# VinAIResearch/Point-Unet

Hardware: AMD Instinct MI355X
Metric: points_per_sec_forward (higher is better)
Workload: dtype f32

## Files before the change

### point-unet_amd/csrc/attpool32b.hip

```cpp
#include "attpool.h"
#include "b3_ops.h"
#include "mfma_tile.h"
#include "wave_ops.h"

namespace ps {

struct Att32bArgs {
    const float* xyz;
    const int32_t* idx;
    const int32_t* order;
    const float* fg;
    const uint4* w1; const float* b1;
    const uint4* w2; const float* b2;
    const uint4* wb;
    float* agg;
    int n_total, n_cloud;
};

__device__ __forceinline__ B3Planes load_planes(const uint4* img, int slot, int lane)
{
    B3Planes r;
    r.p[0] = img[(slot * 3 + 0) * 64 + lane];
    r.p[1] = img[(slot * 3 + 1) * 64 + lane];
    r.p[2] = img[(slot * 3 + 2) * 64 + lane];
    return r;
}

template <int D, int STAGE, int KN, int WAVES>
__global__ __launch_bounds__(WAVES * 64) void att32b_kernel(Att32bArgs a)
{
    constexpr int H = D / 2, LDF = H + D, PITCH = H + 4, PPT = 32 / KN, RP = 16 / PPT;
    constexpr int CBH = H / 32, CBD = D / 32, NQ = H / 16;
    constexpr int W1Q = CBH * 3 * 64, W2Q = STAGE == 2 ? CBH * NQ * 3 * 64 : 0, WBQ = CBD * NQ * 3 * 64;
    constexpr int TILE = 32 * PITCH;
    static_assert(H % 32 == 0 && (KN == 16 || KN == 32), "att32b: d_out >= 64, K in {16, 32}");

    extern __shared__ __attribute__((aligned(16))) float smem[];
    const int wave = __builtin_amdgcn_readfirstlane(threadIdx.x >> 6), lane = threadIdx.x & 63;
    const int hl = lane >> 5, c32 = lane & 31;
    uint4* Wq = reinterpret_cast<uint4*>(smem);
    constexpr int WTOT = (W1Q + W2Q + WBQ) * 4 + 2 * H;
    float* own = smem + WTOT + wave * (32 + TILE);
    int* NB = reinterpret_cast<int*>(own);
    float* T1 = own + 32;
    for (int i = threadIdx.x; i < W1Q; i += WAVES * 64) Wq[i] = a.w1[i];
    for (int i = threadIdx.x; i < W2Q; i += WAVES * 64) Wq[W1Q + i] = a.w2[i];
    for (int i = threadIdx.x; i < WBQ; i += WAVES * 64) Wq[W1Q + W2Q + i] = a.wb[i];
    float* bias = smem + (W1Q + W2Q + WBQ) * 4;
    for (int i = threadIdx.x; i < H; i += WAVES * 64) {
        bias[i] = a.b1[i];
        bias[H + i] = STAGE == 2 ? a.b2[i] : 0.f;
    }
    __syncthreads();
    const uint4 *w1 = Wq, *w2 = Wq + W1Q, *wb = Wq + W1Q + W2Q;
    const float *b1 = bias, *b2 = bias + H;

    const int per_xcd = ((((a.n_total + 7) >> 3) + PPT - 1) / PPT) * PPT;
    const int xcd = blockIdx.x & 7, slot = blockIdx.x >> 3, slots = gridDim.x >> 3;
    const int t_end = min(a.n_total, (xcd + 1) * per_xcd);
    const int t_first = xcd * per_xcd + (slot * WAVES + wave) * PPT, t_step = slots * WAVES * PPT;
    int n_pp[PPT], n_nl = 0;
    float n_c[3], n_n[3];
    const bool one_cloud = a.n_total == a.n_cloud;
    auto cloud_base = [&](int row) { return one_cloud ? 0 : (row / a.n_cloud) * a.n_cloud; };
    auto gstage = [&](int st, int t0n) {
        if (t0n >= t_end) return;
        if (st == 0) {
#pragma unroll
            for (int i = 0; i < PPT; ++i) {
                const int t = min(t0n + i, t_end - 1);
                n_pp[i] = a.order ? cloud_base(t) + a.order[t] : t;
            }
        } else if (st == 1) {
            const unsigned p = PPT == 2 ? (c32 >= KN ? n_pp[PPT - 1] : n_pp[0]) : n_pp[0];
            n_nl = a.idx[p * (unsigned)KN + (unsigned)(c32 & (KN - 1))];
            const float* cp = a.xyz + 3u * p;
            n_c[0] = cp[0]; n_c[1] = cp[1]; n_c[2] = cp[2];
        } else {
            const int p = PPT == 2 ? (c32 >= KN ? n_pp[PPT - 1] : n_pp[0]) : n_pp[0];
            n_nl += cloud_base(p);
            const float* np = a.xyz + 3u * (unsigned)n_nl;
            n_n[0] = np[0]; n_n[1] = np[1]; n_n[2] = np[2];
        }
    };
    gstage(0, t_first);
    gstage(1, t_first);
    gstage(2, t_first);
    for (int t0 = t_first; t0 < t_end; t0 += t_step) {
        int pp[PPT];
#pragma unroll
        for (int i = 0; i < PPT; ++i) pp[i] = n_pp[i];
        const int nbr = n_nl;
        const float cx = n_c[0], cy = n_c[1], cz = n_c[2];
        const float nx = n_n[0], ny = n_n[1], nz = n_n[2];
        const float rx = cx - nx, ry = cy - ny, rz = cz - nz;
        const float dis = __builtin_amdgcn_sqrtf(rx * rx + ry * ry + rz * rz);
        const float ev[8] = {hl ? ny : dis, hl ? nz : rx, hl ? 0.f : ry, hl ? 0.f : rz, hl ? 0.f : cx, hl ? 0.f : cy, hl ? 0.f : cz, hl ? 0.f : nx};
        const B3Planes E = b3_split8<3>(ev);
        if (hl == 0) NB[c32] = nbr;
        gstage(0, t0 + t_step);
        wave_lds_sync();
        unsigned off[16];
        {
            const unsigned col0 = (unsigned)c32 * 4u;
#pragma unroll
            for (int g4 = 0; g4 < 4; ++g4) {
                const int4 nb4 = *reinterpret_cast<const int4*>(NB + 8 * g4 + 4 * hl);
                off[4 * g4] = __umul24(nb4.x, LDF * 4u) + col0; off[4 * g4 + 1] = __umul24(nb4.y, LDF * 4u) + col0;
                off[4 * g4 + 2] = __umul24(nb4.z, LDF * 4u) + col0; off[4 * g4 + 3] = __umul24(nb4.w, LDF * 4u) + col0;
            }
        }
        const char* fgb = reinterpret_cast<const char*>(a.fg);
        f32x2 gq[2][8], v[2][8];
        auto gather = [&](int i, f32x2 (&gdst)[8], f32x2 (&vdst)[8]) {
            const int rel = i * 32 * 4;
#pragma unroll
            for (int r = 0; r < 16; ++r) gdst[r >> 1][r & 1] = *reinterpret_cast<const float*>(fgb + off[r] + (rel + H * 4));
            if (i * 32 < H) {
#pragma unroll
                for (int r = 0; r < 16; ++r) vdst[r >> 1][r & 1] = *reinterpret_cast<const float*>(fgb + off[r] + rel);
            }
        };
        gather(0, gq[0], v[0]);

        f32x16 f1[CBH];
#pragma unroll
        for (int cb = 0; cb < CBH; ++cb) {
            f32x16 acc;
#pragma unroll
            for (int g4 = 0; g4 < 4; ++g4) {
                const float4 bb = *reinterpret_cast<const float4*>(b1 + cb * 32 + g4 * 8 + hl * 4);
                acc[4 * g4] = bb.x; acc[4 * g4 + 1] = bb.y; acc[4 * g4 + 2] = bb.z; acc[4 * g4 + 3] = bb.w;
            }
            acc = b3_mfma6<3>(load_planes(w1, cb, lane), E, acc);
#pragma unroll
            for (int r = 0; r < 16; ++r) f1[cb][r] = leaky02(acc[r]);
        }
        gstage(1, t0 + t_step);
        B3Planes P[NQ];
        auto split_block = [&](const f32x16& f, B3Planes& lo, B3Planes& hi) {
            const float x0[8] = {f[0], f[1], f[2], f[3], f[4], f[5], f[6], f[7]};
            const float x1[8] = {f[8], f[9], f[10], f[11], f[12], f[13], f[14], f[15]};
            lo = b3_split8<3>(x0);
            hi = b3_split8<3>(x1);
        };
        auto store_block = [&](const f32x16& f, int cb) {
#pragma unroll
            for (int g4 = 0; g4 < 4; ++g4) {
                float4 o;
                o.x = f[4 * g4]; o.y = f[4 * g4 + 1]; o.z = f[4 * g4 + 2]; o.w = f[4 * g4 + 3];
                *reinterpret_cast<float4*>(T1 + c32 * PITCH + cb * 32 + g4 * 8 + hl * 4) = o;
            }
        };
#pragma unroll
        for (int cb = 0; cb < CBH; ++cb) split_block(f1[cb], P[2 * cb], P[2 * cb + 1]);
        if constexpr (STAGE == 1) {
#pragma unroll
            for (int cb = 0; cb < CBH; ++cb) store_block(f1[cb], cb);
        } else {
            f32x16 f2[CBH];
#pragma unroll
            for (int cb = 0; cb < CBH; ++cb) {
                f32x16 acc;
#pragma unroll
                for (int g4 = 0; g4 < 4; ++g4) {
                    const float4 bb = *reinterpret_cast<const float4*>(b2 + cb * 32 + g4 * 8 + hl * 4);
                    acc[4 * g4] = bb.x; acc[4 * g4 + 1] = bb.y; acc[4 * g4 + 2] = bb.z; acc[4 * g4 + 3] = bb.w;
                }
#pragma unroll
                for (int q = 0; q < NQ; ++q) acc = b3_mfma6<3>(load_planes(w2, cb * NQ + q, lane), P[q], acc);
#pragma unroll
                for (int r = 0; r < 16; ++r) f2[cb][r] = leaky02(acc[r]);
            }
#pragma unroll
            for (int cb = 0; cb < CBH; ++cb) {
                split_block(f2[cb], P[2 * cb], P[2 * cb + 1]);
                store_block(f2[cb], cb);
            }
        }
        wave_lds_sync();
        const float* TX = T1;

#pragma unroll
        for (int cb = 0; cb < CBD; ++cb) {
            if (cb + 1 < CBD) gather(cb + 1, gq[(cb + 1) & 1], v[(cb + 1) & 1]);
            if (cb == 0) gstage(2, t0 + t_step);
            f32x16 acc;
#pragma unroll
            for (int r = 0; r < 16; ++r) acc[r] = 0.f;
#pragma unroll
            for (int q = 0; q < NQ; ++q) acc = b3_mfma6<3>(P[q], load_planes(wb, cb * NQ + q, lane), acc);
            f32x2 (&vv)[8] = v[cb & 1];
            if (cb * 32 >= H) {
                const float* tv = TX + (cb * 32 - H + c32) + 4 * hl * PITCH;
#pragma unroll
                for (int r = 0; r < 16; ++r) vv[r >> 1][r & 1] = tv[((r & 3) + 8 * (r >> 2)) * PITCH];
            }
            f32x2 sc[8];
            const f32x2 l2e = {1.4426950408889634f, 1.4426950408889634f};
#pragma unroll
            for (int j = 0; j < 8; ++j) sc[j] = __builtin_elementwise_fma(gq[cb & 1][j], l2e, f32x2{acc[2 * j], acc[2 * j + 1]});
            constexpr int PP = RP / 2;
#pragma unroll
            for (int pi = 0; pi < PPT; ++pi) {
                float m = fmaxf(sc[pi * PP][0], sc[pi * PP][1]);
#pragma unroll
                for (int j = 1; j < PP; ++j) m = fmaxf(m, fmaxf(sc[pi * PP + j][0], sc[pi * PP + j][1]));
                m = swap32_max(m);
                const f32x2 mm = {m, m};
                f32x2 ssum2 = {0.f, 0.f}, num2 = {0.f, 0.f};
#pragma unroll
                for (int j = 0; j < PP; ++j) {
                    const f32x2 dd = sc[pi * PP + j] - mm;
                    const f32x2 ex = {__builtin_amdgcn_exp2f(dd[0]), __builtin_amdgcn_exp2f(dd[1])};
                    ssum2 += ex;
                    num2 = __builtin_elementwise_fma(ex, vv[pi * PP + j], num2);
                }
                const float ssum = swap32_sum(ssum2[0] + ssum2[1]);
                const float num = swap32_sum(num2[0] + num2[1]);
                if (hl == 0 && t0 + pi < t_end) a.agg[__umul24(pp[pi], D) + (unsigned)(cb * 32 + c32)] = num * __builtin_amdgcn_rcpf(ssum);
            }
        }
        wave_lds_sync();
    }
}


template <int D, int STAGE, int KN, int WAVES>
__global__ __launch_bounds__(WAVES * 64) void att32s_kernel(Att32bArgs a)
{
    constexpr int H = D / 2, LDF = H + D, PITCH = H + 4, PPT = 32 / KN, RP = 16 / PPT;
    constexpr int CBH = H / 32, CBD = D / 32, NQ = H / 16;
    constexpr int PLQ = NQ * 3 * 64;
    constexpr int NB_H = CBH / WAVES, NB_D = CBD / WAVES;
    static_assert(CBH % WAVES == 0 && NB_D == 2 && (KN == 16 || KN == 32), "att32s: two score blocks per wave");

    extern __shared__ __attribute__((aligned(16))) float smem[];
    const int wave = threadIdx.x >> 6, lane = threadIdx.x & 63;
    const int hl = lane >> 5, c32 = lane & 31;
    int* NB = reinterpret_cast<int*>(smem);
    uint4* PA = reinterpret_cast<uint4*>(smem + 32);
    uint4* PB = STAGE == 2 ? PA + PLQ : PA;
    float* TV = reinterpret_cast<float*>(PB + PLQ);

    const int per_xcd = ((((a.n_total + 7) >> 3) + PPT - 1) / PPT) * PPT;
    const int xcd = blockIdx.x & 7, slot = blockIdx.x >> 3, slots = gridDim.x >> 3;
    const int t_end = min(a.n_total, (xcd + 1) * per_xcd);
    const int t_first = xcd * per_xcd + slot * PPT, t_step = slots * PPT;
    int n_pp[PPT], n_nl = 0;
    float n_c[3], n_n[3];
    const bool one_cloud = a.n_total == a.n_cloud;
    auto cloud_base = [&](int row) { return one_cloud ? 0 : (row / a.n_cloud) * a.n_cloud; };
    auto gstage = [&](int st, int t0n) {
        if (t0n >= t_end) return;
        if (st == 0) {
#pragma unroll
            for (int i = 0; i < PPT; ++i) {
                const int t = min(t0n + i, t_end - 1);
                n_pp[i] = a.order ? cloud_base(t) + a.order[t] : t;
            }
        } else if (st == 1) {
            const unsigned p = PPT == 2 ? (c32 >= KN ? n_pp[PPT - 1] : n_pp[0]) : n_pp[0];
            n_nl = a.idx[p * (unsigned)KN + (unsigned)(c32 & (KN - 1))];
            const float* cp = a.xyz + 3u * p;
            n_c[0] = cp[0]; n_c[1] = cp[1]; n_c[2] = cp[2];
        } else {
            const int p = PPT == 2 ? (c32 >= KN ? n_pp[PPT - 1] : n_pp[0]) : n_pp[0];
            n_nl += cloud_base(p);
            const float* np = a.xyz + 3u * (unsigned)n_nl;
            n_n[0] = np[0]; n_n[1] = np[1]; n_n[2] = np[2];
        }
    };
    auto seed = [&](const float* b, int cb) {
        f32x16 acc;
#pragma unroll
        for (int g4 = 0; g4 < 4; ++g4) {
            const float4 bb = *reinterpret_cast<const float4*>(b + cb * 32 + g4 * 8 + hl * 4);
            acc[4 * g4] = bb.x; acc[4 * g4 + 1] = bb.y; acc[4 * g4 + 2] = bb.z; acc[4 * g4 + 3] = bb.w;
        }
        return acc;
    };
    auto emit_block = [&](const f32x16& acc, int cb, uint4* planes, bool values) {
        float x0[8], x1[8];
#pragma unroll
        for (int r = 0; r < 8; ++r) { x0[r] = leaky02(acc[r]); x1[r] = leaky02(acc[8 + r]); }
        const B3Planes lo = b3_split8<3>(x0), hi = b3_split8<3>(x1);
#pragma unroll
        for (int pl = 0; pl < 3; ++pl) {
            planes[((2 * cb) * 3 + pl) * 64 + lane] = lo.p[pl];
            planes[((2 * cb + 1) * 3 + pl) * 64 + lane] = hi.p[pl];
        }
        if (values) {
#pragma unroll
            for (int g4 = 0; g4 < 4; ++g4) {
                const float* x = g4 < 2 ? x0 + 4 * g4 : x1 + 4 * (g4 - 2);
                *reinterpret_cast<float4*>(TV + c32 * PITCH + cb * 32 + g4 * 8 + hl * 4) = make_float4(x[0], x[1], x[2], x[3]);
            }
        }
    };
    gstage(0, t_first);
    gstage(1, t_first);
    gstage(2, t_first);
    static_assert(NB_H == 1, "att32s: one transposed block per wave");
    const B3Planes W1 = load_planes(a.w1, wave, lane);
    const f32x16 seed1 = seed(a.b1, wave);
    constexpr int PD = D >= 512 ? 4 : 2;
    constexpr int PD2 = STAGE == 2 ? (D >= 512 ? 4 : 8) : 1;
    const int cbA = wave, cbB = wave + WAVES;
    for (int t0 = t_first; t0 < t_end; t0 += t_step) {
        int pp[PPT];
#pragma unroll
        for (int i = 0; i < PPT; ++i) pp[i] = n_pp[i];
        const int nbr = n_nl;
        const float cx = n_c[0], cy = n_c[1], cz = n_c[2];
        const float nx = n_n[0], ny = n_n[1], nz = n_n[2];
        const float rx = cx - nx, ry = cy - ny, rz = cz - nz;
        const float dis = __builtin_amdgcn_sqrtf(rx * rx + ry * ry + rz * rz);
        const float ev[8] = {hl ? ny : dis, hl ? nz : rx, hl ? 0.f : ry, hl ? 0.f : rz, hl ? 0.f : cx, hl ? 0.f : cy, hl ? 0.f : cz, hl ? 0.f : nx};
        const B3Planes E = b3_split8<3>(ev);
        if (hl == 0 && wave == 0) NB[c32] = nbr;
        gstage(0, t0 + t_step);
        B3Planes ring[PD2], rA[PD], rB[PD];
        if constexpr (STAGE == 2) {
#pragma unroll
            for (int q = 0; q < PD2; ++q) ring[q] = load_planes(a.w2, wave * NQ + q, lane);
        } else {
#pragma unroll
            for (int q = 0; q < PD; ++q) {
                rA[q] = load_planes(a.wb, cbA * NQ + q, lane);
                rB[q] = load_planes(a.wb, cbB * NQ + q, lane);
            }
        }

        emit_block(b3_mfma6<3>(W1, E, seed1), wave, PA, STAGE == 1);
        __syncthreads();
        gstage(1, t0 + t_step);
        unsigned off[16];
        {
            const unsigned col0 = (unsigned)(wave * 32 + c32) * 4u;
#pragma unroll
            for (int g4 = 0; g4 < 4; ++g4) {
                const int4 nb4 = *reinterpret_cast<const int4*>(NB + 8 * g4 + 4 * hl);
                off[4 * g4] = __umul24(nb4.x, LDF * 4u) + col0; off[4 * g4 + 1] = __umul24(nb4.y, LDF * 4u) + col0;
                off[4 * g4 + 2] = __umul24(nb4.z, LDF * 4u) + col0; off[4 * g4 + 3] = __umul24(nb4.w, LDF * 4u) + col0;
            }
        }
        const char* fgb = reinterpret_cast<const char*>(a.fg);
        if constexpr (STAGE == 2) {
            const int cb = wave;
            f32x16 acc = seed(a.b2, cb);
#pragma unroll 1
            for (int q0 = 0; q0 + PD2 < NQ; q0 += PD2) {
#pragma unroll
                for (int j = 0; j < PD2; ++j) {
                    acc = b3_mfma6<3>(ring[j], load_planes(PA, q0 + j, lane), acc);
                    ring[j] = load_planes(a.w2, cb * NQ + q0 + j + PD2, lane);
                }
            }
#pragma unroll
            for (int j = 0; j < PD2; ++j) acc = b3_mfma6<3>(ring[j], load_planes(PA, NQ - PD2 + j, lane), acc);
#pragma unroll
            for (int q = 0; q < PD; ++q) {
                rA[q] = load_planes(a.wb, cbA * NQ + q, lane);
                rB[q] = load_planes(a.wb, cbB * NQ + q, lane);
            }
            emit_block(acc, cb, PB, true);
            __syncthreads();
        }
        gstage(2, t0 + t_step);

        f32x16 accA, accB;
#pragma unroll
        for (int r = 0; r < 16; ++r) { accA[r] = 0.f; accB[r] = 0.f; }
        f32x2 gq[2][8], v[2][8];
        {
#pragma unroll 1
            for (int q0 = 0; q0 + PD < NQ; q0 += PD) {
#pragma unroll
                for (int j = 0; j < PD; ++j) {
                    const B3Planes x = load_planes(PB, q0 + j, lane);
                    accA = b3_mfma6<3>(x, rA[j], accA);
                    accB = b3_mfma6<3>(x, rB[j], accB);
                    rA[j] = load_planes(a.wb, cbA * NQ + q0 + j + PD, lane);
                    rB[j] = load_planes(a.wb, cbB * NQ + q0 + j + PD, lane);
                }
            }
#pragma unroll
            for (int i = 0; i < 2; ++i)
#pragma unroll
                for (int r = 0; r < 16; ++r) gq[i][r >> 1][r & 1] = *reinterpret_cast<const float*>(fgb + off[r] + (i * WAVES * 32 * 4 + H * 4));
#pragma unroll
            for (int j = 0; j < PD; ++j) {
                const B3Planes x = load_planes(PB, NQ - PD + j, lane);
                accA = b3_mfma6<3>(x, rA[j], accA);
                accB = b3_mfma6<3>(x, rB[j], accB);
            }
        }
#pragma unroll
        for (int r = 0; r < 16; ++r) v[0][r >> 1][r & 1] = *reinterpret_cast<const float*>(fgb + off[r]);
#pragma unroll
        for (int ii = 0; ii < 2; ++ii) {
            const int i = 1 - ii;
            const int cb = wave + i * WAVES;
            const f32x16& acc = i == 0 ? accA : accB;
            f32x2 (&vv)[8] = v[i];
            if (cb * 32 >= H) {
                const float* tv = TV + (cb * 32 - H + c32) + 4 * hl * PITCH;
#pragma unroll
                for (int r = 0; r < 16; ++r) vv[r >> 1][r & 1] = tv[((r & 3) + 8 * (r >> 2)) * PITCH];
            }
            f32x2 sc[8];
            const f32x2 l2e = {1.4426950408889634f, 1.4426950408889634f};
#pragma unroll
            for (int j = 0; j < 8; ++j) sc[j] = __builtin_elementwise_fma(gq[i][j], l2e, f32x2{acc[2 * j], acc[2 * j + 1]});
            constexpr int PP = RP / 2;
#pragma unroll
            for (int pi = 0; pi < PPT; ++pi) {
                float m = fmaxf(sc[pi * PP][0], sc[pi * PP][1]);
#pragma unroll
                for (int j = 1; j < PP; ++j) m = fmaxf(m, fmaxf(sc[pi * PP + j][0], sc[pi * PP + j][1]));
                m = swap32_max(m);
                const f32x2 mm = {m, m};
                f32x2 ssum2 = {0.f, 0.f}, num2 = {0.f, 0.f};
#pragma unroll
                for (int j = 0; j < PP; ++j) {
                    const f32x2 dd = sc[pi * PP + j] - mm;
                    const f32x2 ex = {__builtin_amdgcn_exp2f(dd[0]), __builtin_amdgcn_exp2f(dd[1])};
                    ssum2 += ex;
                    num2 = __builtin_elementwise_fma(ex, vv[pi * PP + j], num2);
                }
                const float ssum = swap32_sum(ssum2[0] + ssum2[1]);
                const float num = swap32_sum(num2[0] + num2[1]);
                if (hl == 0 && t0 + pi < t_end) a.agg[__umul24(pp[pi], D) + (unsigned)(cb * 32 + c32)] = num * __builtin_amdgcn_rcpf(ssum);
            }
        }
        __syncthreads();
    }
}

static inline int kmap(int q, int g, int j)
{
    const int r = 8 * (q & 1) + j;
    return 32 * (q >> 1) + (r & 3) + 8 * (r >> 2) + 4 * g;
}

void pack_b3(const float* W, int cin, int cout, uint16_t* out)
{
    const int nq = cin / 16, cbs = cout / 32;
    for (int cb = 0; cb < cbs; ++cb)
        for (int q = 0; q < nq; ++q)
            for (int pl = 0; pl < 3; ++pl)
                for (int l = 0; l < 64; ++l)
                    for (int j = 0; j < 8; ++j)
                        out[(((((size_t)cb * nq + q) * 3 + pl) * 64 + l) * 8) + j] = b3_piece_of(W[(size_t)kmap(q, l >> 5, j) * cout + 32 * cb + (l & 31)], pl);
}

void pack_b3_locse(const float* W1, int cout, uint16_t* out)
{
    const int cbs = cout / 32;
    for (int cb = 0; cb < cbs; ++cb)
        for (int pl = 0; pl < 3; ++pl)
            for (int l = 0; l < 64; ++l)
                for (int j = 0; j < 8; ++j) {
                    const int k = 8 * (l >> 5) + j;
                    out[((((size_t)cb * 3 + pl) * 64 + l) * 8) + j] = k < 10 ? b3_piece_of(W1[(size_t)k * cout + 32 * cb + (l & 31)], pl) : (uint16_t)0;
                }
}

template <int D, int STAGE, int KN>
static int launch_att32b(ps_context* c, const Att32bArgs& a)
{
    constexpr int H = D / 2, PITCH = H + 4, TILE = 32 * PITCH;
    constexpr int CBH = H / 32, CBD = D / 32, NQ = H / 16;
    constexpr int WAVES = D == 128 ? 8 : (STAGE == 1 ? 16 : 12);
    constexpr int PER_CU = 1;
    constexpr size_t planes = (size_t)(CBH + (STAGE == 2 ? CBH * NQ : 0) + CBD * NQ) * 3 * 64 * 16;
    constexpr size_t smem = planes + sizeof(float) * (2 * H + (size_t)WAVES * (32 + TILE));
    static_assert(smem <= 160 * 1024, "att32b: weights + tiles exceed the LDS");
    auto kern = att32b_kernel<D, STAGE, KN, WAVES>;
    PS_HIP(hipFuncSetAttribute(reinterpret_cast<const void*>(kern), hipFuncAttributeMaxDynamicSharedMemorySize, (int)smem));
    const int tiles = ceil_div(a.n_total, 32 / KN);
    const int blocks = (std::min(ceil_div(tiles, WAVES), 256 * PER_CU) + 7) & ~7;
    hipLaunchKernelGGL(kern, dim3(blocks), dim3(WAVES * 64), smem, c->stream, a);
    PS_HIP(hipGetLastError());
    return PS_OK;
}

template <int D, int STAGE, int KN>
static int launch_att32s(ps_context* c, const Att32bArgs& a)
{
    constexpr int H = D / 2, PITCH = H + 4, NQ = H / 16;
    constexpr int WAVES = D / 64;
    constexpr size_t smem = sizeof(float) * 32 + (size_t)(STAGE == 2 ? 2 : 1) * NQ * 3 * 64 * 16 + sizeof(float) * 32 * PITCH;
    static_assert(smem <= 160 * 1024, "att32s: planes + value tile exceed the LDS");
    auto kern = att32s_kernel<D, STAGE, KN, WAVES>;
    if (smem > 48 * 1024) PS_HIP(hipFuncSetAttribute(reinterpret_cast<const void*>(kern), hipFuncAttributeMaxDynamicSharedMemorySize, (int)smem));
    const int tiles = ceil_div(a.n_total, 32 / KN);
    const int blocks = (std::min(tiles, 256 * 16) + 7) & ~7;
    hipLaunchKernelGGL(kern, dim3(blocks), dim3(WAVES * 64), smem, c->stream, a);
    PS_HIP(hipGetLastError());
    return PS_OK;
}

bool att_pool32b_fits(const AttStage& s)
{
    return att_pool32_fits(s) && s.p32->w1b && (s.d == 64 || s.d == 128 || s.d == 256 || s.d == 512);
}

int att_pool32b_stage(ps_context* c, const AttStage& s)
{
    Att32bArgs a;
    a.xyz = s.xyz; a.idx = s.idx; a.order = s.order; a.fg = s.fg;
    a.w1 = reinterpret_cast<const uint4*>(s.p32->w1b); a.b1 = s.lfa1->bias;
    a.w2 = s.lfa2 ? reinterpret_cast<const uint4*>(s.p32->w2b) : nullptr; a.b2 = s.lfa2 ? s.lfa2->bias : nullptr;
    a.wb = reinterpret_cast<const uint4*>(s.lfa2 ? s.p32->wb2b : s.p32->wb1b);
    a.agg = s.agg;
    a.n_total = (int)s.n_total; a.n_cloud = (int)s.n_cloud;
    if (s.n_total <= 0) return PS_OK;
    const int stage = s.lfa2 ? 2 : 1;
#define PS_A32B(DD)                                                                                                      \
    if (s.k == 16) return stage == 1 ? launch_att32b<DD, 1, 16>(c, a) : launch_att32b<DD, 2, 16>(c, a);                  \
    return stage == 1 ? launch_att32b<DD, 1, 32>(c, a) : launch_att32b<DD, 2, 32>(c, a)
    if (s.d == 64) { PS_A32B(64); }
    if (s.d == 128) { PS_A32B(128); }
#undef PS_A32B
#define PS_A32S(DD)                                                                                                      \
    if (s.k == 16) return stage == 1 ? launch_att32s<DD, 1, 16>(c, a) : launch_att32s<DD, 2, 16>(c, a);                  \
    return stage == 1 ? launch_att32s<DD, 1, 32>(c, a) : launch_att32s<DD, 2, 32>(c, a)
    if (s.d == 256) { PS_A32S(256); }
    PS_A32S(512);
#undef PS_A32S
}

}
```

Measured before the change: 193.5 million.

## Process two point tiles per iteration in att32s to reuse weight planes

The att32s attention-pool kernel now handles T (default 2) point tiles per loop iteration, so each weight plane loaded from global memory feeds MFMAs for several tiles. The per-block value tile is replaced by a small per-wave scratch that transposes values into registers, and the separate second plane buffer is dropped. Neighbour gathers are interleaved with the softmax/aggregation work. Launch bounds now request two blocks per CU and the grid is sized per XCD group. The cost is higher register pressure from doubled accumulators and more LDS for per-tile planes.

```diff
diff --git a/point-unet_amd/csrc/attpool32b.hip b/point-unet_amd/csrc/attpool32b.hip
--- a/point-unet_amd/csrc/attpool32b.hip
+++ b/point-unet_amd/csrc/attpool32b.hip
@@ -226,10 +226,10 @@
 }
 
 
-template <int D, int STAGE, int KN, int WAVES>
-__global__ __launch_bounds__(WAVES * 64) void att32s_kernel(Att32bArgs a)
-{
-    constexpr int H = D / 2, LDF = H + D, PITCH = H + 4, PPT = 32 / KN, RP = 16 / PPT;
+template <int D, int STAGE, int KN, int WAVES, int T>
+__global__ __launch_bounds__(WAVES * 64, 2) void att32s_kernel(Att32bArgs a)
+{
+    constexpr int H = D / 2, LDF = H + D, SCP = 36, PPT = 32 / KN, RP = 16 / PPT;
     constexpr int CBH = H / 32, CBD = D / 32, NQ = H / 16;
     constexpr int PLQ = NQ * 3 * 64;
     constexpr int NB_H = CBH / WAVES, NB_D = CBD / WAVES;
@@ -239,36 +239,47 @@
     const int wave = threadIdx.x >> 6, lane = threadIdx.x & 63;
     const int hl = lane >> 5, c32 = lane & 31;
     int* NB = reinterpret_cast<int*>(smem);
-    uint4* PA = reinterpret_cast<uint4*>(smem + 32);
-    uint4* PB = STAGE == 2 ? PA + PLQ : PA;
-    float* TV = reinterpret_cast<float*>(PB + PLQ);
+    uint4* PA = reinterpret_cast<uint4*>(smem + T * 32);
+    float* SC = reinterpret_cast<float*>(PA + T * PLQ) + wave * (32 * SCP);
 
     const int per_xcd = ((((a.n_total + 7) >> 3) + PPT - 1) / PPT) * PPT;
     const int xcd = blockIdx.x & 7, slot = blockIdx.x >> 3, slots = gridDim.x >> 3;
     const int t_end = min(a.n_total, (xcd + 1) * per_xcd);
-    const int t_first = xcd * per_xcd + slot * PPT, t_step = slots * PPT;
-    int n_pp[PPT], n_nl = 0;
-    float n_c[3], n_n[3];
+    const int t_first = xcd * per_xcd + slot * (T * PPT), t_step = slots * (T * PPT);
+    int n_pp[T][PPT], n_nl[T];
+    float n_c[T][3], n_n[T][3];
+#pragma unroll
+    for (int u = 0; u < T; ++u) {
+        n_nl[u] = 0;
+#pragma unroll
+        for (int i = 0; i < PPT; ++i) n_pp[u][i] = 0;
+#pragma unroll
+        for (int i = 0; i < 3; ++i) { n_c[u][i] = 0.f; n_n[u][i] = 0.f; }
+    }
     const bool one_cloud = a.n_total == a.n_cloud;
     auto cloud_base = [&](int row) { return one_cloud ? 0 : (row / a.n_cloud) * a.n_cloud; };
-    auto gstage = [&](int st, int t0n) {
-        if (t0n >= t_end) return;
-        if (st == 0) {
-#pragma unroll
-            for (int i = 0; i < PPT; ++i) {
-                const int t = min(t0n + i, t_end - 1);
-                n_pp[i] = a.order ? cloud_base(t) + a.order[t] : t;
-            }
-        } else if (st == 1) {
-            const unsigned p = PPT == 2 ? (c32 >= KN ? n_pp[PPT - 1] : n_pp[0]) : n_pp[0];
-            n_nl = a.idx[p * (unsigned)KN + (unsigned)(c32 & (KN - 1))];
-            const float* cp = a.xyz + 3u * p;
-            n_c[0] = cp[0]; n_c[1] = cp[1]; n_c[2] = cp[2];
-        } else {
-            const int p = PPT == 2 ? (c32 >= KN ? n_pp[PPT - 1] : n_pp[0]) : n_pp[0];
-            n_nl += cloud_base(p);
-            const float* np = a.xyz + 3u * (unsigned)n_nl;
-            n_n[0] = np[0]; n_n[1] = np[1]; n_n[2] = np[2];
+    auto gstage = [&](int st, int g0n) {
+#pragma unroll
+        for (int u = 0; u < T; ++u) {
+            const int t0n = g0n + u * PPT;
+            if (t0n >= t_end) continue;
+            if (st == 0) {
+#pragma unroll
+                for (int i = 0; i < PPT; ++i) {
+                    const int t = min(t0n + i, t_end - 1);
+                    n_pp[u][i] = a.order ? cloud_base(t) + a.order[t] : t;
+                }
+            } else if (st == 1) {
+                const unsigned p = PPT == 2 ? (c32 >= KN ? n_pp[u][PPT - 1] : n_pp[u][0]) : n_pp[u][0];
+                n_nl[u] = a.idx[p * (unsigned)KN + (unsigned)(c32 & (KN - 1))];
+                const float* cp = a.xyz + 3u * p;
+                n_c[u][0] = cp[0]; n_c[u][1] = cp[1]; n_c[u][2] = cp[2];
+            } else {
+                const int p = PPT == 2 ? (c32 >= KN ? n_pp[u][PPT - 1] : n_pp[u][0]) : n_pp[u][0];
+                n_nl[u] += cloud_base(p);
+                const float* np = a.xyz + 3u * (unsigned)n_nl[u];
+                n_n[u][0] = np[0]; n_n[u][1] = np[1]; n_n[u][2] = np[2];
+            }
         }
     };
     auto seed = [&](const float* b, int cb) {
@@ -280,7 +291,7 @@
         }
         return acc;
     };
-    auto emit_block = [&](const f32x16& acc, int cb, uint4* planes, bool values) {
+    auto emit_block = [&](const f32x16& acc, int cb, uint4* planes, bool values, f32x2 (&vout)[8]) {
         float x0[8], x1[8];
 #pragma unroll
         for (int r = 0; r < 8; ++r) { x0[r] = leaky02(acc[r]); x1[r] = leaky02(acc[8 + r]); }
@@ -294,31 +305,40 @@
 #pragma unroll
             for (int g4 = 0; g4 < 4; ++g4) {
                 const float* x = g4 < 2 ? x0 + 4 * g4 : x1 + 4 * (g4 - 2);
-                *reinterpret_cast<float4*>(TV + c32 * PITCH + cb * 32 + g4 * 8 + hl * 4) = make_float4(x[0], x[1], x[2], x[3]);
-            }
+                *reinterpret_cast<float4*>(SC + c32 * SCP + g4 * 8 + hl * 4) = make_float4(x[0], x[1], x[2], x[3]);
+            }
+            wave_lds_sync();
+            const float* tv = SC + c32 + 4 * hl * SCP;
+#pragma unroll
+            for (int r = 0; r < 16; ++r) vout[r >> 1][r & 1] = tv[((r & 3) + 8 * (r >> 2)) * SCP];
+            wave_lds_sync();
         }
     };
     gstage(0, t_first);
     gstage(1, t_first);
     gstage(2, t_first);
     static_assert(NB_H == 1, "att32s: one transposed block per wave");
-    const B3Planes W1 = load_planes(a.w1, wave, lane);
-    const f32x16 seed1 = seed(a.b1, wave);
-    constexpr int PD = D >= 512 ? 4 : 2;
-    constexpr int PD2 = STAGE == 2 ? (D >= 512 ? 4 : 8) : 1;
+    B3Planes W1 = load_planes(a.w1, wave, lane);
+    f32x16 seed1 = seed(a.b1, wave);
+    constexpr int PD = T >= 2 ? 2 : (D >= 512 ? 4 : 2);
+    constexpr int PD2 = STAGE == 2 ? (T >= 2 ? 2 : (D >= 512 ? 4 : 8)) : 1;
     const int cbA = wave, cbB = wave + WAVES;
+    const char* fgb = reinterpret_cast<const char*>(a.fg);
     for (int t0 = t_first; t0 < t_end; t0 += t_step) {
-        int pp[PPT];
-#pragma unroll
-        for (int i = 0; i < PPT; ++i) pp[i] = n_pp[i];
-        const int nbr = n_nl;
-        const float cx = n_c[0], cy = n_c[1], cz = n_c[2];
-        const float nx = n_n[0], ny = n_n[1], nz = n_n[2];
-        const float rx = cx - nx, ry = cy - ny, rz = cz - nz;
-        const float dis = __builtin_amdgcn_sqrtf(rx * rx + ry * ry + rz * rz);
-        const float ev[8] = {hl ? ny : dis, hl ? nz : rx, hl ? 0.f : ry, hl ? 0.f : rz, hl ? 0.f : cx, hl ? 0.f : cy, hl ? 0.f : cz, hl ? 0.f : nx};
-        const B3Planes E = b3_split8<3>(ev);
-        if (hl == 0 && wave == 0) NB[c32] = nbr;
+        int pp[T][PPT];
+        B3Planes E[T];
+#pragma unroll
+        for (int u = 0; u < T; ++u) {
+#pragma unroll
+            for (int i = 0; i < PPT; ++i) pp[u][i] = n_pp[u][i];
+            const float cx = n_c[u][0], cy = n_c[u][1], cz = n_c[u][2];
+            const float nx = n_n[u][0], ny = n_n[u][1], nz = n_n[u][2];
+            const float rx = cx - nx, ry = cy - ny, rz = cz - nz;
+            const float dis = __builtin_amdgcn_sqrtf(rx * rx + ry * ry + rz * rz);
+            const float ev[8] = {hl ? ny : dis, hl ? nz : rx, hl ? 0.f : ry, hl ? 0.f : rz, hl ? 0.f : cx, hl ? 0.f : cy, hl ? 0.f : cz, hl ? 0.f : nx};
+            E[u] = b3_split8<3>(ev);
+            if (hl == 0 && wave == 0) NB[u * 32 + c32] = n_nl[u];
+        }
         gstage(0, t0 + t_step);
         B3Planes ring[PD2], rA[PD], rB[PD];
         if constexpr (STAGE == 2) {
@@ -332,87 +352,103 @@
             }
         }
 
-        emit_block(b3_mfma6<3>(W1, E, seed1), wave, PA, STAGE == 1);
+        f32x2 vB[T][8];
+#pragma unroll
+        for (int u = 0; u < T; ++u) emit_block(b3_mfma6<3>(W1, E[u], seed1), wave, PA + u * PLQ, STAGE == 1, vB[u]);
         __syncthreads();
         gstage(1, t0 + t_step);
-        unsigned off[16];
-        {
-            const unsigned col0 = (unsigned)(wave * 32 + c32) * 4u;
-#pragma unroll
-            for (int g4 = 0; g4 < 4; ++g4) {
-                const int4 nb4 = *reinterpret_cast<const int4*>(NB + 8 * g4 + 4 * hl);
-                off[4 * g4] = __umul24(nb4.x, LDF * 4u) + col0; off[4 * g4 + 1] = __umul24(nb4.y, LDF * 4u) + col0;
-                off[4 * g4 + 2] = __umul24(nb4.z, LDF * 4u) + col0; off[4 * g4 + 3] = __umul24(nb4.w, LDF * 4u) + col0;
-            }
-        }
-        const char* fgb = reinterpret_cast<const char*>(a.fg);
         if constexpr (STAGE == 2) {
             const int cb = wave;
-            f32x16 acc = seed(a.b2, cb);
+            f32x16 acc[T];
+#pragma unroll
+            for (int u = 0; u < T; ++u) acc[u] = seed(a.b2, cb);
 #pragma unroll 1
             for (int q0 = 0; q0 + PD2 < NQ; q0 += PD2) {
 #pragma unroll
                 for (int j = 0; j < PD2; ++j) {
-                    acc = b3_mfma6<3>(ring[j], load_planes(PA, q0 + j, lane), acc);
+#pragma unroll
+                    for (int u = 0; u < T; ++u) acc[u] = b3_mfma6<3>(ring[j], load_planes(PA + u * PLQ, q0 + j, lane), acc[u]);
                     ring[j] = load_planes(a.w2, cb * NQ + q0 + j + PD2, lane);
                 }
             }
 #pragma unroll
-            for (int j = 0; j < PD2; ++j) acc = b3_mfma6<3>(ring[j], load_planes(PA, NQ - PD2 + j, lane), acc);
+            for (int j = 0; j < PD2; ++j)
+#pragma unroll
+                for (int u = 0; u < T; ++u) acc[u] = b3_mfma6<3>(ring[j], load_planes(PA + u * PLQ, NQ - PD2 + j, lane), acc[u]);
 #pragma unroll
             for (int q = 0; q < PD; ++q) {
                 rA[q] = load_planes(a.wb, cbA * NQ + q, lane);
                 rB[q] = load_planes(a.wb, cbB * NQ + q, lane);
             }
-            emit_block(acc, cb, PB, true);
             __syncthreads();
+#pragma unroll
+            for (int u = 0; u < T; ++u) emit_block(acc[u], cb, PA + u * PLQ, true, vB[u]);
+            __syncthreads();
         }
         gstage(2, t0 + t_step);
 
-        f32x16 accA, accB;
-#pragma unroll
-        for (int r = 0; r < 16; ++r) { accA[r] = 0.f; accB[r] = 0.f; }
-        f32x2 gq[2][8], v[2][8];
-        {
+        f32x16 accA[T], accB[T];
+#pragma unroll
+        for (int u = 0; u < T; ++u)
+#pragma unroll
+            for (int r = 0; r < 16; ++r) { accA[u][r] = 0.f; accB[u][r] = 0.f; }
 #pragma unroll 1
-            for (int q0 = 0; q0 + PD < NQ; q0 += PD) {
-#pragma unroll
-                for (int j = 0; j < PD; ++j) {
-                    const B3Planes x = load_planes(PB, q0 + j, lane);
-                    accA = b3_mfma6<3>(x, rA[j], accA);
-                    accB = b3_mfma6<3>(x, rB[j], accB);
-                    rA[j] = load_planes(a.wb, cbA * NQ + q0 + j + PD, lane);
-                    rB[j] = load_planes(a.wb, cbB * NQ + q0 + j + PD, lane);
-                }
-            }
-#pragma unroll
-            for (int i = 0; i < 2; ++i)
-#pragma unroll
-                for (int r = 0; r < 16; ++r) gq[i][r >> 1][r & 1] = *reinterpret_cast<const float*>(fgb + off[r] + (i * WAVES * 32 * 4 + H * 4));
+        for (int q0 = 0; q0 + PD < NQ; q0 += PD) {
 #pragma unroll
             for (int j = 0; j < PD; ++j) {
-                const B3Planes x = load_planes(PB, NQ - PD + j, lane);
-                accA = b3_mfma6<3>(x, rA[j], accA);
-                accB = b3_mfma6<3>(x, rB[j], accB);
-            }
-        }
-#pragma unroll
-        for (int r = 0; r < 16; ++r) v[0][r >> 1][r & 1] = *reinterpret_cast<const float*>(fgb + off[r]);
-#pragma unroll
-        for (int ii = 0; ii < 2; ++ii) {
-            const int i = 1 - ii;
+#pragma unroll
+                for (int u = 0; u < T; ++u) {
+                    const B3Planes x = load_planes(PA + u * PLQ, q0 + j, lane);
+                    accA[u] = b3_mfma6<3>(x, rA[j], accA[u]);
+                    accB[u] = b3_mfma6<3>(x, rB[j], accB[u]);
+                }
+                rA[j] = load_planes(a.wb, cbA * NQ + q0 + j + PD, lane);
+                rB[j] = load_planes(a.wb, cbB * NQ + q0 + j + PD, lane);
+            }
+        }
+        f32x2 gq[2][8], v0[8];
+        auto gather = [&](int k) {
+            const int u = k >> 1, i = 1 - (k & 1);
+            const unsigned col0 = (unsigned)(wave * 32 + c32) * 4u;
+            unsigned off[16];
+#pragma unroll
+            for (int g4 = 0; g4 < 4; ++g4) {
+                const int4 nb4 = *reinterpret_cast<const int4*>(NB + u * 32 + 8 * g4 + 4 * hl);
+                off[4 * g4] = __umul24(nb4.x, LDF * 4u) + col0; off[4 * g4 + 1] = __umul24(nb4.y, LDF * 4u) + col0;
+                off[4 * g4 + 2] = __umul24(nb4.z, LDF * 4u) + col0; off[4 * g4 + 3] = __umul24(nb4.w, LDF * 4u) + col0;
+            }
+#pragma unroll
+            for (int r = 0; r < 16; ++r) gq[k & 1][r >> 1][r & 1] = *reinterpret_cast<const float*>(fgb + off[r] + (i * WAVES * 32 * 4 + H * 4));
+            if (i == 0) {
+#pragma unroll
+                for (int r = 0; r < 16; ++r) v0[r >> 1][r & 1] = *reinterpret_cast<const float*>(fgb + off[r]);
+            }
+        };
+#pragma unroll
+        for (int j = 0; j < PD; ++j) {
+#pragma unroll
+            for (int u = 0; u < T; ++u) {
+                const B3Planes x = load_planes(PA + u * PLQ, NQ - PD + j, lane);
+                accA[u] = b3_mfma6<3>(x, rA[j], accA[u]);
+                accB[u] = b3_mfma6<3>(x, rB[j], accB[u]);
+            }
+            if (j == 0) gather(0);
+        }
+#pragma unroll
+        for (int k = 0; k < 2 * T; ++k) {
+            if (k + 1 < 2 * T) gather(k + 1);
+            if (k == 2 * T - 2) {
+                W1 = load_planes(a.w1, wave, lane);
+                seed1 = seed(a.b1, wave);
+            }
+            const int u = k >> 1, i = 1 - (k & 1);
             const int cb = wave + i * WAVES;
-            const f32x16& acc = i == 0 ? accA : accB;
-            f32x2 (&vv)[8] = v[i];
-            if (cb * 32 >= H) {
-                const float* tv = TV + (cb * 32 - H + c32) + 4 * hl * PITCH;
-#pragma unroll
-                for (int r = 0; r < 16; ++r) vv[r >> 1][r & 1] = tv[((r & 3) + 8 * (r >> 2)) * PITCH];
-            }
+            const f32x16& acc = i == 0 ? accA[u] : accB[u];
+            const f32x2 (&vv)[8] = i == 0 ? v0 : vB[u];
             f32x2 sc[8];
             const f32x2 l2e = {1.4426950408889634f, 1.4426950408889634f};
 #pragma unroll
-            for (int j = 0; j < 8; ++j) sc[j] = __builtin_elementwise_fma(gq[i][j], l2e, f32x2{acc[2 * j], acc[2 * j + 1]});
+            for (int j = 0; j < 8; ++j) sc[j] = __builtin_elementwise_fma(gq[k & 1][j], l2e, f32x2{acc[2 * j], acc[2 * j + 1]});
             constexpr int PP = RP / 2;
 #pragma unroll
             for (int pi = 0; pi < PPT; ++pi) {
@@ -431,7 +467,7 @@
                 }
                 const float ssum = swap32_sum(ssum2[0] + ssum2[1]);
                 const float num = swap32_sum(num2[0] + num2[1]);
-                if (hl == 0 && t0 + pi < t_end) a.agg[__umul24(pp[pi], D) + (unsigned)(cb * 32 + c32)] = num * __builtin_amdgcn_rcpf(ssum);
+                if (hl == 0 && t0 + u * PPT + pi < t_end) a.agg[__umul24(pp[u][pi], D) + (unsigned)(cb * 32 + c32)] = num * __builtin_amdgcn_rcpf(ssum);
             }
         }
         __syncthreads();
@@ -486,17 +522,22 @@
     return PS_OK;
 }
 
+#ifndef PS_ATT32S_TILES
+#define PS_ATT32S_TILES 2
+#endif
+
 template <int D, int STAGE, int KN>
 static int launch_att32s(ps_context* c, const Att32bArgs& a)
 {
-    constexpr int H = D / 2, PITCH = H + 4, NQ = H / 16;
+    constexpr int H = D / 2, NQ = H / 16, PPT = 32 / KN, T = PS_ATT32S_TILES;
     constexpr int WAVES = D / 64;
-    constexpr size_t smem = sizeof(float) * 32 + (size_t)(STAGE == 2 ? 2 : 1) * NQ * 3 * 64 * 16 + sizeof(float) * 32 * PITCH;
-    static_assert(smem <= 160 * 1024, "att32s: planes + value tile exceed the LDS");
-    auto kern = att32s_kernel<D, STAGE, KN, WAVES>;
+    constexpr size_t smem = sizeof(float) * 32 * T + (size_t)T * NQ * 3 * 64 * 16 + sizeof(float) * WAVES * 32 * 36;
+    static_assert(smem <= 160 * 1024, "att32s: planes + scratch exceed the LDS");
+    auto kern = att32s_kernel<D, STAGE, KN, WAVES, T>;
     if (smem > 48 * 1024) PS_HIP(hipFuncSetAttribute(reinterpret_cast<const void*>(kern), hipFuncAttributeMaxDynamicSharedMemorySize, (int)smem));
-    const int tiles = ceil_div(a.n_total, 32 / KN);
-    const int blocks = (std::min(tiles, 256 * 16) + 7) & ~7;
+    const int per_xcd = ceil_div(ceil_div(a.n_total, 8), PPT) * PPT;
+    const int groups = ceil_div(per_xcd / PPT, T);
+    const int blocks = 8 * std::min(groups, 512);
     hipLaunchKernelGGL(kern, dim3(blocks), dim3(WAVES * 64), smem, c->stream, a);
     PS_HIP(hipGetLastError());
     return PS_OK;
```

Result: no change. 195.1 million (median of 6 runs) (+0.9%).
